# csiro-robotics/ohm

Measured on AMD Instinct MI355X. Metric: rays/sec integrated (occupancy), higher is better.
Workload: dtype f64

## Files before the change

### ohm_amd/csrc/occupancy_math.h

```cpp
#ifndef OHMHIP_OCCUPANCY_MATH_H
#define OHMHIP_OCCUPANCY_MATH_H

#include "walk_device.h"

namespace ohmhip
{
__device__ inline float fInf()
{
  return __int_as_float(0x7f800000);
}

__device__ inline bool sameValue(float a, float b)
{
  return __float_as_uint(a) == __float_as_uint(b);
}

__device__ inline float occMiss(const MapConst &mc, unsigned ray_flags, float initial)
{
  const float inf = fInf();
  const bool unobserved = initial == inf;
  const bool is_free = !unobserved && initial < mc.threshold_value;
  const bool is_occ = !unobserved && initial >= mc.threshold_value;
  float adj = mc.miss_value;
  adj = (unobserved && (ray_flags & OHMHIP_RF_EXCLUDE_UNOBSERVED)) ? inf : adj;
  adj = (is_free && (ray_flags & OHMHIP_RF_EXCLUDE_FREE)) ? 0.0f : adj;
  adj = (is_occ && (ray_flags & OHMHIP_RF_EXCLUDE_OCCUPIED)) ? 0.0f : adj;
  const float base = unobserved ? 0.0f : initial;
  adj = (unobserved || (mc.sat_min < initial && initial < mc.sat_max)) ? adj : 0.0f;
  return (base != inf) ? fmaxf(mc.min_value, base + adj) : base;
}

__device__ inline float occHit(const MapConst &mc, unsigned ray_flags, float initial)
{
  const float inf = fInf();
  const bool unobserved = initial == inf;
  const bool is_free = !unobserved && initial < mc.threshold_value;
  const bool is_occ = !unobserved && initial >= mc.threshold_value;
  float adj = mc.hit_value;
  adj = (unobserved && (ray_flags & OHMHIP_RF_EXCLUDE_UNOBSERVED)) ? inf : adj;
  adj = (is_free && (ray_flags & OHMHIP_RF_EXCLUDE_FREE)) ? 0.0f : adj;
  adj = (is_occ && (ray_flags & OHMHIP_RF_EXCLUDE_OCCUPIED)) ? 0.0f : adj;
  const float base = unobserved ? 0.0f : initial;
  adj = (unobserved || (mc.sat_min < initial && initial < mc.sat_max)) ? adj : 0.0f;
  return (base != inf) ? fminf(base + adj, mc.max_value) : base;
}

__device__ inline float occNullMiss(const MapConst &mc, float initial)
{
  return (initial != fInf()) ? fmaxf(mc.min_value, initial + 0.0f) : initial;
}

__device__ inline float occMissN(const MapConst &mc, unsigned ray_flags, float x, uint32_t n)
{
  constexpr unsigned kExcludeFlags = OHMHIP_RF_EXCLUDE_UNOBSERVED | OHMHIP_RF_EXCLUDE_FREE | OHMHIP_RF_EXCLUDE_OCCUPIED;
  if (n == 0)
  {
    return x;
  }
  if (!(ray_flags & kExcludeFlags))
  {
    const bool unobserved = x == fInf();
    const float base = unobserved ? 0.0f : x;
    const float first_adj = (unobserved || (mc.sat_min < x && x < mc.sat_max)) ? mc.miss_value : 0.0f;
    float nx = fmaxf(mc.min_value, base + first_adj);
    if (nx == x)
    {
      return nx;
    }
    x = nx;
    for (uint32_t k = 1; k < n; ++k)
    {
      const float adj = (mc.sat_min < x && x < mc.sat_max) ? mc.miss_value : 0.0f;
      nx = fmaxf(mc.min_value, x + adj);
      const bool fixed = nx == x;
      x = nx;
      if (fixed)
      {
        break;
      }
    }
    return x;
  }
  for (uint32_t k = 0; k < n; ++k)
  {
    const float nx = occMiss(mc, ray_flags, x);
    const bool fixed = nx == x;
    x = nx;
    if (fixed)
    {
      break;
    }
  }
  return x;
}

__device__ inline uint32_t subVoxelUpdate(uint32_t coord, uint32_t point_count, const double v[3], double resolution)
{
  const int mean_positions = (1 << 10) - 1;
  const double mean_resolution = resolution / double(mean_positions);
  const double offset = double(0.5f) * resolution;
  double mean[3];
  mean[0] = int(coord & mean_positions) * mean_resolution - offset;
  mean[1] = int((coord >> 10) & mean_positions) * mean_resolution - offset;
  mean[2] = int((coord >> 20) & mean_positions) * mean_resolution - offset;
  const double one_on_count_plus_one = double(1) / double(point_count + 1);
  uint32_t pattern = 0;
#pragma unroll
  for (int a = 0; a < 3; ++a)
  {
    mean[a] += (v[a] - mean[a]) * one_on_count_plus_one;
    int pos = pointToRegionCoord(mean[a] + offset, mean_resolution);
    pos = (pos >= 0 ? (pos < (1 << 10) ? pos : mean_positions) : 0);
    pattern |= uint32_t(pos) << (10 * a);
  }
  return pattern | (1u << 31);
}
}

#endif
```

### ohm_amd/csrc/walk_kernel.h

```cpp
#ifndef OHMHIP_WALK_KERNEL_H
#define OHMHIP_WALK_KERNEL_H

#include "batch_scratch.h"
#include "occupancy_math.h"
#include "region_table.h"
#include "walk_device.h"

namespace ohmhip
{
constexpr int kWalkThreads = 1024;
constexpr int kWalkWaves = kWalkThreads / 64;
constexpr int kQueueCap = 128;
#ifndef OHMHIP_LDS_HITS
#define OHMHIP_LDS_HITS 6144
#endif
constexpr int kLdsHits = OHMHIP_LDS_HITS;
constexpr uint32_t kIndexShift = 5;
constexpr uint32_t kIndexBuckets = (1u << kHitVoxelBits) >> kIndexShift;
constexpr int kRefillMinIdle = 20;
constexpr uint32_t kTileFlag = 0x8000u;
constexpr uint32_t kTileCountMask = 0x7fffu;
#ifndef OHMHIP_MAX_CHUNK_SEGMENTS
#define OHMHIP_MAX_CHUNK_SEGMENTS 8192
#endif
constexpr uint32_t kMaxChunkSegments = OHMHIP_MAX_CHUNK_SEGMENTS;
constexpr uint32_t kTraceChunks = 4096;
constexpr uint32_t kTraceWords = 32;
constexpr uint32_t kLengthClasses = 128;

__device__ inline uint32_t tileWord(uint32_t w)
{
  return w ^ (((w >> 5) ^ (w >> 10)) & 31u);
}

__device__ inline uint32_t tileAddress(uint32_t va)
{
  return (va & ~3u) ^ ((((va >> 5) ^ (va >> 10)) & (31u << 2)));
}

__device__ inline void resolveFlaggedMiss(unsigned long long key, const BatchScratch &bs,
                                          const unsigned long long *__restrict__ sorted_hits,
                                          uint32_t *__restrict__ miss_counts, uint32_t *__restrict__ interval_counts,
                                          int region_voxels)
{
  const uint32_t slot = hitSlot(key);
  const uint32_t vi = hitVoxel(key);
  const uint32_t he = bs.info->n_hits;
  uint32_t lo = bs.voxel_first_hit[size_t(slot) * size_t(region_voxels) + vi];
  while (lo < he && hitGroup(sorted_hits[lo]) == hitGroup(key) && sorted_hits[lo] < key)
  {
    ++lo;
  }
  if (lo < he && hitGroup(sorted_hits[lo]) == hitGroup(key))
  {
    atomicAdd(&interval_counts[lo], 1u);
    atomicSub(&miss_counts[size_t(slot) * size_t(region_voxels) + vi], 1u);
  }
}

__device__ inline void flushQueue(const uint2 *queue, uint32_t qcount, unsigned lane, unsigned long long slot_bits,
                                  int ray_shift, bool lds_resolve, const unsigned long long *l_hits,
                                  const uint16_t *l_index, uint32_t n_region_hits, uint32_t *l_intervals,
                                  uint32_t *l_counts,
                                  unsigned long long *__restrict__ events, uint32_t event_capacity,
                                  uint32_t *__restrict__ event_count, int defer_all, const BatchScratch &bs,
                                  const unsigned long long *__restrict__ sorted_hits,
                                  uint32_t *__restrict__ miss_counts, uint32_t *__restrict__ interval_counts,
                                  int region_voxels)
{
  if (lds_resolve)
  {
    for (uint32_t q = lane; q < qcount; q += 64)
    {
      const uint2 e = queue[q];
      const unsigned long long ev =
        slot_bits | ((unsigned long long)e.x << kHitRayBits) | ((unsigned long long)e.y << ray_shift);
      uint32_t lo = l_index[e.x >> kIndexShift], hi = l_index[(e.x >> kIndexShift) + 1u];
      while (lo < hi)
      {
        const uint32_t mid = (lo + hi) >> 1;
        if (l_hits[mid] > ev)
        {
          hi = mid;
        }
        else
        {
          lo = mid + 1;
        }
      }
      if (lo < n_region_hits && hitGroup(l_hits[lo]) == hitGroup(ev))
      {
        atomicAdd(&l_intervals[lo >> 1], 1u << ((lo & 1u) * 16u));
        atomicSub(&l_counts[tileWord(e.x >> 1)], 1u << ((e.x & 1u) * 16u));
      }
    }
    return;
  }
  uint32_t gbase = 0;
  if (lane == 0)
  {
    gbase = atomicAdd(event_count, qcount);
  }
  gbase = __shfl(gbase, 0);
  for (uint32_t q = lane; q < qcount; q += 64)
  {
    const uint2 e = queue[q];
    const unsigned long long ev =
      slot_bits | ((unsigned long long)e.x << kHitRayBits) | ((unsigned long long)e.y << ray_shift);
    if (gbase + q < event_capacity)
    {
      events[gbase + q] = ev;
    }
    else if (!defer_all)
    {
      resolveFlaggedMiss(ev, bs, sorted_hits, miss_counts, interval_counts, region_voxels);
    }
  }
}

constexpr int kFcmpOlt = 4;
constexpr int kIcmpSlt = 40;

__device__ inline int selectI(unsigned long long mask, int if_set, int if_clear)
{
  int r;
  asm("v_cndmask_b32_e64 %0, %1, %2, %3" : "=v"(r) : "v"(if_clear), "v"(if_set), "s"(mask));
  return r;
}

__device__ inline double selectD(unsigned long long mask, double if_set, double if_clear)
{
  const int lo = selectI(mask, __double2loint(if_set), __double2loint(if_clear));
  const int hi = selectI(mask, __double2hiint(if_set), __double2hiint(if_clear));
  return __hiloint2double(hi, lo);
}

__device__ inline int addMask(int value, unsigned long long mask)
{
  asm("v_addc_co_u32_e64 %0, vcc, 0, %0, %1" : "+v"(value) : "s"(mask) : "vcc");
  return value;
}

constexpr int kIcmpEq = 32;
constexpr int kIcmpUlt = 36;

__device__ inline uint32_t selectOrZero(unsigned long long mask, uint32_t if_set)
{
  uint32_t r;
  asm("v_cndmask_b32_e64 %0, 0, %1, %2" : "=v"(r) : "v"(if_set), "s"(mask));
  return r;
}

__device__ inline uint32_t umin3(uint32_t a, uint32_t b, uint32_t c)
{
  uint32_t r;
  asm("v_min3_u32 %0, %1, %2, %3" : "=v"(r) : "v"(a), "v"(b), "v"(c));
  return r;
}

__device__ inline uint32_t umed3(uint32_t a, uint32_t b, uint32_t c)
{
  uint32_t r;
  asm("v_med3_u32 %0, %1, %2, %3" : "=v"(r) : "v"(a), "v"(b), "v"(c));
  return r;
}

__device__ inline uint32_t addSat(uint32_t a, uint32_t b)
{
  uint32_t r;
  asm("v_add_u32_e64 %0, %1, %2 clamp" : "=v"(r) : "v"(a), "v"(b));
  return r;
}

__device__ inline uint32_t addSatUniform(uint32_t a, uint32_t b)
{
  uint32_t r;
  asm("v_add_u32_e64 %0, %1, %2 clamp" : "=v"(r) : "v"(a), "s"(b));
  return r;
}

__device__ inline uint32_t tileAdd(uint32_t byte_address, uint32_t value)
{
  uint32_t old;
  asm volatile("ds_add_rtn_u32 %0, %1, %2" : "=v"(old) : "v"(byte_address), "v"(value) : "memory");
  return old;
}

__device__ inline uint32_t shiftOne(uint32_t shift)
{
  uint32_t r;
  asm("v_lshlrev_b32_e64 %0, %1, 1" : "=v"(r) : "v"(shift));
  return r;
}

__device__ inline uint32_t waitTile(uint32_t old)
{
  asm volatile("s_waitcnt lgkmcnt(0)" : "+v"(old) : : "memory");
  return old;
}

struct WalkArgs
{
  MapConst mc;
  BatchScratch bs;
  const Chunk *chunks;
  const Segment *segments;
  const RayWalk *walks;
  const uint64_t *slot_keys;
  const unsigned long long *sorted_hits;
  const uint32_t *hit_mask;
  uint32_t *miss_counts;
  uint32_t *interval_counts;
  unsigned long long *events;
  uint32_t event_capacity;
  uint32_t *event_count;
  int refill_min_idle;
  unsigned dbg;
  int ray_shift;
  int defer_all;
  float *occupancy;
  unsigned ray_flags;
  unsigned long long *dbg_counters;
  float *tsdf;
  uint32_t *chunk_cursor;
  uint32_t n_chunks;
  int rewalk;
  int flag_all;
  int inline_hits;
};

constexpr uint32_t kWalkCursorWords = 24;
#ifndef OHMHIP_WALK_UNROLL
#define OHMHIP_WALK_UNROLL 2
#endif
constexpr int kWalkUnroll = OHMHIP_WALK_UNROLL;

template <int kThreadsT, int kTileVoxelsT, int kLdsHitsT, uint32_t kSegmentsT, int kQueueCapT, int kMinWavesPerEuT>
struct WalkGeometry
{
  static constexpr int kMinWavesPerEu = kMinWavesPerEuT;
  static constexpr int kThreads = kThreadsT;
  static constexpr int kWaves = kThreadsT / 64;
  static constexpr int kTileVoxels = kTileVoxelsT;
  static constexpr int kLdsHits = kLdsHitsT;
  static constexpr uint32_t kSegments = kSegmentsT;
  static constexpr int kQueueCap = kQueueCapT;
};
using WalkFull = WalkGeometry<kWalkThreads, 1 << kHitVoxelBits, kLdsHits, kMaxChunkSegments, kQueueCap, 1>;
using WalkHalf = WalkGeometry<kWalkThreads / 2, (1 << kHitVoxelBits) / 2, kLdsHits / 2, kMaxChunkSegments / 2, 96, 4>;
template <bool kSpecial, bool kTrace, typename G = WalkFull>
__global__ void __launch_bounds__(G::kThreads, G::kMinWavesPerEu) k_region_walk(WalkArgs args)
{
  extern __shared__ __attribute__((aligned(16))) uint32_t lds[];
  const MapConst &mc = args.mc;
  const uint32_t count_words = uint32_t(mc.region_voxels + 1) >> 1;
  const uint32_t mask_words = uint32_t(mc.region_voxels + 31) >> 5;
  uint32_t *l_counts = lds;
  uint2 *l_queues = reinterpret_cast<uint2 *>(lds + ((count_words + 31u) & ~31u));
  unsigned long long *l_hits = reinterpret_cast<unsigned long long *>(l_queues + G::kWaves * G::kQueueCap);
  uint32_t *l_intervals = reinterpret_cast<uint32_t *>(l_hits + G::kLdsHits);
  uint32_t *l_cursor = l_intervals + G::kLdsHits / 2;
  uint32_t *l_hist = l_cursor + kWalkCursorWords;
  uint32_t *l_idle = l_hist + kLengthClasses;
  uint16_t *l_index = reinterpret_cast<uint16_t *>(l_idle + 64);
  uint16_t *l_order = l_index + kIndexBuckets + 2;

  const int defer_all = args.defer_all;
  auto fetchNextChunk = [&](uint32_t *record, bool first = false) {
    const uint32_t next = first ? blockIdx.x : gridDim.x + atomicAdd(args.chunk_cursor, 1u);
    record[1] = next;
    if (next < args.n_chunks)
    {
      const Chunk c = args.chunks[next];
      record[2] = c.slot;
      record[3] = c.seg_begin;
      record[4] = c.seg_end;
      record[5] = c.hash_index;
      record[6] = defer_all ? 0u : args.bs.hit_begin[c.slot];
      record[7] = defer_all ? 0u : args.bs.hit_end[c.slot];
      const uint64_t key = args.slot_keys[c.slot];
      record[8] = uint32_t(key);
      record[9] = uint32_t(key >> 32);
    }
  };
  constexpr int kSegPerThread = int(G::kSegments) / G::kThreads;
  constexpr int kHitsPerThread = G::kLdsHits / uint32_t(G::kThreads);
  struct ChunkRecord
  {
    uint32_t index, slot, seg_begin, seg_end, hash_index, hb, he, key_lo, key_hi;
  };
  auto readRecord = [&](const uint32_t *record) {
    ChunkRecord r;
    r.index = __builtin_amdgcn_readfirstlane(record[1]);
    r.slot = __builtin_amdgcn_readfirstlane(record[2]);
    r.seg_begin = __builtin_amdgcn_readfirstlane(record[3]);
    r.seg_end = __builtin_amdgcn_readfirstlane(record[4]);
    r.hash_index = __builtin_amdgcn_readfirstlane(record[5]);
    r.hb = __builtin_amdgcn_readfirstlane(record[6]);
    r.he = __builtin_amdgcn_readfirstlane(record[7]);
    r.key_lo = __builtin_amdgcn_readfirstlane(record[8]);
    r.key_hi = __builtin_amdgcn_readfirstlane(record[9]);
    return r;
  };
  unsigned long long pf_hits[kHitsPerThread] = {};
  uint32_t pf_vox[kSegPerThread] = {};
  uint32_t pf_mask = 0;
  auto prefetchChunk = [&](const ChunkRecord &r) {
    const uint32_t n_hits = r.he - r.hb;
    if (!defer_all && n_hits && n_hits <= uint32_t(G::kLdsHits))
    {
#pragma unroll
      for (int j = 0; j < kHitsPerThread; ++j)
      {
        pf_hits[j] = args.sorted_hits[r.hb + min(threadIdx.x + uint32_t(j) * uint32_t(G::kThreads), n_hits - 1u)];
      }
    }
    pf_mask = args.hit_mask[size_t(r.slot) * mask_words + min(threadIdx.x, mask_words - 1u)];
    const uint32_t n = r.seg_end - r.seg_begin;
#pragma unroll
    for (int j = 0; j < kSegPerThread; ++j)
    {
      pf_vox[j] = args.segments[r.seg_begin + min(threadIdx.x + uint32_t(j) * uint32_t(G::kThreads), n - 1u)].vox;
    }
  };
  if (threadIdx.x == 0 || threadIdx.x == 64)
  {
    fetchNextChunk(l_cursor + (threadIdx.x ? kWalkCursorWords / 2 : 0), threadIdx.x == 0);
  }
  __syncthreads();
  ChunkRecord cur = readRecord(l_cursor);
  ChunkRecord next = readRecord(l_cursor + kWalkCursorWords / 2);
  if (next.index < cur.index)
  {
    const ChunkRecord swap = cur;
    cur = next;
    next = swap;
  }
  if (cur.index < args.n_chunks)
  {
    prefetchChunk(cur);
  }
  __syncthreads();
  while (cur.index < args.n_chunks)
  {
    unsigned long long clk_start = 0;
    if (kTrace)
    {
      clk_start = wall_clock64();
    }
    const uint32_t chunk_index = cur.index;
    Chunk chunk;
    chunk.slot = cur.slot;
    chunk.seg_begin = cur.seg_begin;
    chunk.seg_end = cur.seg_end;
    chunk.hash_index = cur.hash_index;
    const uint32_t hb = cur.hb;
    const uint32_t he = cur.he;
    const int region_x = int(int16_t(cur.key_lo & 0xffffu));
    const int region_y = int(int16_t(cur.key_lo >> 16));
    const int region_z = int(int16_t(cur.key_hi & 0xffffu));
    const uint32_t n_seg = chunk.seg_end - chunk.seg_begin;
    const Segment *chunk_segments = args.segments + chunk.seg_begin;

    const uint32_t n_region_hits = he - hb;
    const bool lds_resolve = !defer_all && n_region_hits <= uint32_t(G::kLdsHits);
    unsigned long long my_hits[kHitsPerThread];
#pragma unroll
    for (int j = 0; j < kHitsPerThread; ++j)
    {
      my_hits[j] = pf_hits[j];
    }
    const uint32_t *g_mask = args.hit_mask + size_t(chunk.slot) * mask_words;
    const uint32_t my_mask = pf_mask;
    uint32_t lens[kSegPerThread];
#pragma unroll
    for (int j = 0; j < kSegPerThread; ++j)
    {
      lens[j] = min(pf_vox[j] >> kSegVoxelBits, kLengthClasses - 1u);
    }
    if (threadIdx.x < kLengthClasses)
    {
      l_hist[threadIdx.x] = 0;
    }
    if (threadIdx.x == 0)
    {
      l_cursor[0] = 0;
    }
    if (threadIdx.x < 64)
    {
      l_idle[threadIdx.x] = 0;
    }
    const bool stamp = kTrace && threadIdx.x == 0;
    unsigned long long clk_p[6] = { 0, 0, 0, 0, 0, 0 };
    if (stamp)
    {
      clk_p[0] = wall_clock64();
    }
    for (uint32_t w = threadIdx.x; w < mask_words; w += uint32_t(G::kThreads))
    {
      const uint32_t mword = args.flag_all ? 0xffffffffu : ((w == threadIdx.x) ? my_mask : g_mask[w]);
      const uint32_t swizzle = tileWord(w * 16u) ^ (w * 16u);
#pragma unroll
      for (uint32_t q = 0; q < 4; ++q)
      {
        const uint32_t logical = w * 16u + q * 4u;
        if (logical + 3u < count_words)
        {
          uint32_t v[4];
#pragma unroll
          for (uint32_t r = 0; r < 4; ++r)
          {
            const uint32_t two = (mword >> ((q * 4u + (r ^ (swizzle & 3u))) * 2u)) & 3u;
            v[r] = ((two & 1u) << 15) | ((two & 2u) << 30);
          }
          *reinterpret_cast<uint4 *>(&l_counts[logical ^ (swizzle & ~3u)]) = make_uint4(v[0], v[1], v[2], v[3]);
        }
        else
        {
          for (uint32_t r = 0; r < 4; ++r)
          {
            if (logical + r < count_words)
            {
              const uint32_t two = (mword >> ((q * 4u + r) * 2u)) & 3u;
              l_counts[tileWord(logical + r)] = ((two & 1u) << 15) | ((two & 2u) << 30);
            }
          }
        }
      }
    }
    if (stamp)
    {
      clk_p[1] = wall_clock64();
    }
    __syncthreads();
    bool prefetched = false;
    if (stamp)
    {
      clk_p[2] = wall_clock64();
    }
#pragma unroll
    for (int j = 0; j < kSegPerThread; ++j)
    {
      if (threadIdx.x + uint32_t(j) * uint32_t(G::kThreads) < n_seg)
      {
        atomicAdd(&l_hist[lens[j]], 1u);
      }
    }
    if (lds_resolve && n_region_hits)
    {
#pragma unroll
      for (int j = 0; j < kHitsPerThread; ++j)
      {
        const uint32_t i = threadIdx.x + uint32_t(j) * uint32_t(G::kThreads);
        if (i < n_region_hits)
        {
          l_hits[i] = my_hits[j];
        }
        if (i < (n_region_hits + 1) / 2)
        {
          l_intervals[i] = 0;
        }
      }
    }
    __syncthreads();
    if (stamp)
    {
      clk_p[3] = wall_clock64();
    }
    if (lds_resolve && n_region_hits)
    {
#pragma unroll
      for (int j = 0; j < kHitsPerThread; ++j)
      {
        const uint32_t i = threadIdx.x + uint32_t(j) * uint32_t(G::kThreads);
        if (i < n_region_hits)
        {
          auto bucketOf = [](unsigned long long key) {
            return (uint32_t(key >> kHitRayBits) & ((1u << kHitVoxelBits) - 1u)) >> kIndexShift;
          };
          const uint32_t b = bucketOf(my_hits[j]);
          const uint32_t first = (i == 0) ? 0u : bucketOf(l_hits[i - 1]) + 1u;
          for (uint32_t k = first; k <= b; ++k)
          {
            l_index[k] = uint16_t(i);
          }
          if (i + 1 == n_region_hits)
          {
            for (uint32_t k = b + 1u; k <= kIndexBuckets; ++k)
            {
              l_index[k] = uint16_t(n_region_hits);
            }
          }
        }
      }
    }
    if (threadIdx.x < 64)
    {
      const uint32_t hi_class = kLengthClasses - 1u - 2u * threadIdx.x;
      const uint32_t a = l_hist[hi_class];
      const uint32_t b = l_hist[hi_class - 1u];
      uint32_t incl = a + b;
#pragma unroll
      for (int d = 1; d < 64; d <<= 1)
      {
        const uint32_t up = __shfl_up(incl, d);
        incl += (int(threadIdx.x) >= d) ? up : 0u;
      }
      const uint32_t excl = incl - (a + b);
      l_hist[hi_class] = excl;
      l_hist[hi_class - 1u] = excl + a;
    }
    __syncthreads();
#pragma unroll
    for (int j = 0; j < kSegPerThread; ++j)
    {
      const uint32_t i = threadIdx.x + uint32_t(j) * uint32_t(G::kThreads);
      if (i < n_seg)
      {
        l_order[atomicAdd(&l_hist[lens[j]], 1u)] = uint16_t(i);
      }
    }
    __syncthreads();
    if (stamp)
    {
      clk_p[4] = wall_clock64();
      if (chunk_index < kTraceChunks)
      {
        unsigned long long *rec = args.dbg_counters + 16 + size_t(chunk_index) * kTraceWords;
        rec[20] = clk_p[0];
        rec[21] = clk_p[1];
        rec[22] = clk_p[2];
        rec[23] = clk_p[3];
      }
    }

    const unsigned lane = laneId();
    const unsigned wave = threadIdx.x >> 6;
    uint2 *queue = l_queues + wave * G::kQueueCap;
    const int dimx = mc.dim[0];
    const int dimxy = mc.dim[0] * mc.dim[1];
    const unsigned long long slot_bits = (unsigned long long)chunk.slot << kHitSlotShift;
    const int ray_shift = args.ray_shift;
    const int refill_min_idle = args.refill_min_idle;
    const bool refill_only = kTrace && (args.dbg & 16u) != 0;
    const uint32_t fix_margin = mc.fix_margin;
    const uint32_t idle_address = uint32_t(reinterpret_cast<char *>(l_idle + lane) - reinterpret_cast<char *>(lds));

    int left = 0;
    uint32_t f0 = 0, f1 = 0, f2 = 0, d0 = 0, d1 = 0, d2 = 0;
    int sx = 0, sy = 0, sz = 0;
    uint32_t va = 0;
    uint32_t ray = 0;
    uint32_t skip = 0;
    uint32_t end_last = 0;
    uint32_t qcount = 0;
    bool exhausted = false;
    uint32_t dbg_iters = 0, dbg_active = 0, dbg_refills = 0, dbg_fm = 0, dbg_slow = 0;
    uint32_t dbg_s2 = 0, dbg_s3 = 0, dbg_sl = 0, dbg_sp = 0;
    unsigned long long clk_loop = 0;
    if (kTrace)
    {
      clk_loop = wall_clock64();
    }

    int refill_threshold = refill_min_idle;
    while (true)
    {
      const unsigned long long am = __ballot(left > 0);
      const int n_idle = 64 - __popcll(am);
      if (__builtin_expect(n_idle >= refill_threshold, 0))
      {
        if (exhausted)
        {
          break;
        }
        if (kTrace)
        {
          ++dbg_refills;
        }
        uint32_t base = 0;
        if (lane == 0)
        {
          base = atomicAdd(l_cursor, uint32_t(n_idle));
        }
        base = __builtin_amdgcn_readfirstlane(base);
        exhausted = base + uint32_t(n_idle) >= n_seg;
        refill_threshold = exhausted ? 64 : refill_threshold;
        const unsigned long long idle = ~am;
        const uint32_t mine =
          base + __builtin_amdgcn_mbcnt_hi(uint32_t(idle >> 32), __builtin_amdgcn_mbcnt_lo(uint32_t(idle), 0u));
        if (left <= 0 && mine < n_seg)
        {
          const uint4 *rec = reinterpret_cast<const uint4 *>(chunk_segments + l_order[mine]);
          const uint4 ra = rec[0];
          const uint4 rb = rec[1];
          f0 = ra.x;
          f1 = ra.y;
          f2 = ra.z;
          va = (ra.w & ((1u << kSegVoxelBits) - 1u)) << 1;
          left = int(ra.w >> kSegVoxelBits);
          d0 = rb.x & ~kSegNegative;
          d1 = rb.y & ~kSegNegative;
          d2 = rb.z & ~kSegNegative;
          sx = (rb.x & kSegNegative) ? -2 : 2;
          sy = (rb.y & kSegNegative) ? -2 * dimx : 2 * dimx;
          sz = (rb.z & kSegNegative) ? -2 * dimxy : 2 * dimxy;
          ray = rb.w & kSegRayMask;
          if (kSpecial)
          {
            skip = (rb.w & kSegSkipFirst) ? 1u : 0u;
            end_last = (rb.w & kSegEnd) ? 1u : 0u;
          }
          left = refill_only ? 0 : left;
        }
        if (!prefetched)
        {
          prefetched = true;
          if (next.index < args.n_chunks)
          {
            prefetchChunk(next);
          }
        }
      }

      uint32_t olds[kWalkUnroll];
      uint32_t visited[kWalkUnroll];
#pragma unroll
      for (int u = 0; u < kWalkUnroll; ++u)
      {
        const bool at_end = kSpecial && end_last && left == 1;
        const bool visit = kSpecial ? (left > 0 && (at_end || !skip)) : (left > 0);
        visited[u] = va;
        olds[u] = tileAdd(visit ? tileAddress(va) : idle_address, shiftOne(va << 3));
        if (kSpecial)
        {
          skip = 0;
        }
        if (kTrace)
        {
          ++dbg_iters;
          dbg_active += uint32_t(__popcll(__ballot(visit)));
        }

        int stride;
        {
          const uint32_t fmin = umin3(f0, f1, f2);
          const uint32_t fmed = umed3(f0, f1, f2);
          const uint32_t limit = min(fmed, kFixMaxDelta);
          const uint32_t lead = addSatUniform(fmin, fix_margin);
          const unsigned long long certain = __builtin_amdgcn_uicmp(lead, limit, kIcmpUlt);
          unsigned long long a0 = __builtin_amdgcn_uicmp(f0, fmin, kIcmpEq);
          unsigned long long a2 = __builtin_amdgcn_uicmp(f2, fmin, kIcmpEq);
          const unsigned long long slow = __ballot(left > 1) & ~certain;
          if (__builtin_expect(slow != 0, 0))
          {
            int axis = 1;
            if ((slow >> lane) & 1ull)
            {
              uint32_t r = ray;
              asm volatile("" : "+v"(r));
              axis = exactNextAxis(mc, args.walks[r], region_x, region_y, region_z, va >> 1);
            }
            a0 = (a0 & ~slow) | (slow & __ballot(axis == 0));
            a2 = (a2 & ~slow) | (slow & __ballot(axis == 2));
            if (kTrace)
            {
              ++dbg_slow;
              dbg_s2 += uint32_t(__popcll(slow & __ballot(left == 2)));
              dbg_s3 += uint32_t(__popcll(slow & __ballot(left == 3)));
              dbg_sl += uint32_t(__popcll(slow));
              dbg_sp += uint32_t(__popcll(slow & __ballot((d0 | d1 | d2) == 0u)));
            }
          }
          const unsigned long long a1 = ~(a0 | a2);
          f0 = addSat(f0, selectOrZero(a0, d0));
          f1 = addSat(f1, selectOrZero(a1, d1));
          f2 = addSat(f2, selectOrZero(a2, d2));
          stride = selectI(a2, sz, selectI(a0, sx, sy));
        }
        va += uint32_t(stride);
        left -= 1;
      }

      __builtin_amdgcn_sched_barrier(0);
#pragma unroll
      for (int u = 0; u < kWalkUnroll; ++u)
      {
        olds[u] = waitTile(olds[u]);
      }
#pragma unroll
      for (int u = 0; u < kWalkUnroll; ++u)
      {
        const bool flagged = __builtin_amdgcn_ubfe(olds[u], (visited[u] << 3) | 15u, 1u) != 0;
        const unsigned long long fm = __ballot(flagged);
        if (kTrace)
        {
          dbg_fm += fm ? 1u : 0u;
        }
        if (fm)
        {
          if (flagged)
          {
            const uint32_t pos =
              qcount + __builtin_amdgcn_mbcnt_hi(uint32_t(fm >> 32), __builtin_amdgcn_mbcnt_lo(uint32_t(fm), 0u));
            queue[pos] = make_uint2(visited[u] >> 1, ray);
          }
          qcount += uint32_t(__popcll(fm));
          if (qcount > uint32_t(G::kQueueCap - 64))
          {
            flushQueue(queue, qcount, lane, slot_bits, ray_shift, lds_resolve, l_hits, l_index, n_region_hits,
                       l_intervals, l_counts, args.events, args.event_capacity, args.event_count, defer_all, args.bs,
                       args.sorted_hits, args.miss_counts, args.interval_counts, mc.region_voxels);
            qcount = 0;
          }
        }
      }
    }

    if (kTrace && lane == 0)
    {
      const unsigned long long clk_end_loop = wall_clock64();
      if (chunk_index < kTraceChunks)
      {
        unsigned long long *rec = args.dbg_counters + 16 + size_t(chunk_index) * kTraceWords;
        if (wave < 15)
        {
          rec[2 + wave] = clk_end_loop;
        }
        if (wave == 0)
        {
          rec[0] = n_seg | ((unsigned long long)((chunk.hash_index >> 31) & 1u) << 32);
          rec[1] = clk_loop;
          rec[18] = clk_start;
          rec[17] = (unsigned long long)__builtin_amdgcn_s_getreg(63492) |
                    ((unsigned long long)__builtin_amdgcn_s_getreg(63508) << 32);
        }
      }
      if (args.dbg & 128u)
      {
        atomicAdd(&args.dbg_counters[0], (unsigned long long)dbg_iters);
        atomicAdd(&args.dbg_counters[1], (unsigned long long)dbg_active);
        atomicAdd(&args.dbg_counters[2], (unsigned long long)dbg_refills);
        atomicAdd(&args.dbg_counters[3], (unsigned long long)dbg_fm);
        atomicAdd(&args.dbg_counters[4], (unsigned long long)dbg_slow);
        atomicAdd(&args.dbg_counters[5], (unsigned long long)dbg_s2);
        atomicAdd(&args.dbg_counters[6], (unsigned long long)dbg_s3);
        atomicAdd(&args.dbg_counters[7], (unsigned long long)dbg_sl);
        atomicAdd(&args.dbg_counters[8], (unsigned long long)dbg_sp);
      }
    }
    if (qcount)
    {
      flushQueue(queue, qcount, lane, slot_bits, ray_shift, lds_resolve, l_hits, l_index, n_region_hits, l_intervals,
                 l_counts, args.events, args.event_capacity, args.event_count, defer_all, args.bs, args.sorted_hits,
                 args.miss_counts, args.interval_counts, mc.region_voxels);
    }
    if (threadIdx.x == 0)
    {
      fetchNextChunk(l_cursor);
    }
    __syncthreads();
    const ChunkRecord after_next = readRecord(l_cursor);
    if (stamp && chunk_index < kTraceChunks)
    {
      args.dbg_counters[16 + size_t(chunk_index) * kTraceWords + 24] = wall_clock64();
    }

    const bool inline_hits = args.inline_hits && lds_resolve && n_region_hits > 0u && args.occupancy && !args.rewalk &&
                             (chunk.hash_index & 0x80000000u);
    if (lds_resolve && !inline_hits)
    {
      for (uint32_t i = threadIdx.x; i < n_region_hits; i += uint32_t(G::kThreads))
      {
        const uint32_t c = (l_intervals[i >> 1] >> ((i & 1u) * 16u)) & 0xffffu;
        if (c)
        {
          atomicAdd(&args.interval_counts[hb + i], c);
        }
      }
    }
    uint32_t *g_counts = args.miss_counts + size_t(chunk.slot) * size_t(mc.region_voxels);
    if (args.rewalk && (chunk.hash_index & 0x80000000u))
    {
      __syncthreads();
      cur = next;
      next = after_next;
      continue;
    }
    if (args.occupancy && (chunk.hash_index & 0x80000000u))
    {
      float *g_occ = args.occupancy + size_t(chunk.slot) * size_t(mc.region_voxels);
      constexpr uint32_t kWordsPerThread = uint32_t(G::kTileVoxels) / 2u / uint32_t(G::kThreads) / 2u;
      const bool even_voxels = (mc.region_voxels & 1) == 0;
      for (uint32_t half = 0; half < 2u; ++half)
      {
      uint32_t words[kWordsPerThread];
      float2 values[kWordsPerThread];
#pragma unroll
      for (uint32_t j = 0; j < kWordsPerThread; ++j)
      {
        const uint32_t i = threadIdx.x + (half * kWordsPerThread + j) * uint32_t(G::kThreads);
        const uint32_t flagged_w = (i < count_words) ? l_counts[tileWord(i)] : 0u;
        uint32_t w = flagged_w;
        w = (w & kTileFlag) ? (w & 0xffff0000u) : w;
        w = (w & (kTileFlag << 16)) ? (w & 0x0000ffffu) : w;
        if (!defer_all && !inline_hits)
        {
          if ((flagged_w & kTileFlag) && (flagged_w & kTileCountMask))
          {
            atomicAdd(&g_counts[2 * i], flagged_w & kTileCountMask);
          }
          if ((flagged_w & (kTileFlag << 16)) && ((flagged_w >> 16) & kTileCountMask))
          {
            atomicAdd(&g_counts[2 * i + 1], (flagged_w >> 16) & kTileCountMask);
          }
        }
        words[j] = w;
        values[j] = make_float2(0.0f, 0.0f);
        if (w)
        {
          if (even_voxels)
          {
            values[j] = *reinterpret_cast<const float2 *>(&g_occ[2 * i]);
          }
          else
          {
            values[j].x = g_occ[2 * i];
            values[j].y = (2 * i + 1 < uint32_t(mc.region_voxels)) ? g_occ[2 * i + 1] : 0.0f;
          }
        }
      }
#pragma unroll
      for (uint32_t j = 0; j < kWordsPerThread; ++j)
      {
        const uint32_t i = threadIdx.x + (half * kWordsPerThread + j) * uint32_t(G::kThreads);
        const uint32_t w = words[j];
        if (w)
        {
          const uint32_t n0 = w & kTileCountMask;
          const uint32_t n1 = (w >> 16) & kTileCountMask;
          if (n0)
          {
            const float v = occMissN(mc, args.ray_flags, values[j].x, n0);
            if (!sameValue(v, values[j].x))
            {
              g_occ[2 * i] = v;
            }
          }
          if (n1)
          {
            const float v = occMissN(mc, args.ray_flags, values[j].y, n1);
            if (!sameValue(v, values[j].y))
            {
              g_occ[2 * i + 1] = v;
            }
          }
        }
      }
      if (stamp && chunk_index < kTraceChunks)
      {
        args.dbg_counters[16 + size_t(chunk_index) * kTraceWords + 25 + half] = wall_clock64();
      }
      }
      if (inline_hits)
      {
        for (uint32_t i = threadIdx.x; i < n_region_hits; i += uint32_t(G::kThreads))
        {
          const unsigned long long key = l_hits[i];
          const unsigned long long group = key >> kHitRayBits;
          if (i > 0u && (l_hits[i - 1u] >> kHitRayBits) == group)
          {
            continue;
          }
          const uint32_t vi = uint32_t(group) & ((1u << kHitVoxelBits) - 1u);
          float x = g_occ[vi];
          for (uint32_t j = i; j < n_region_hits && (l_hits[j] >> kHitRayBits) == group; ++j)
          {
            x = occMissN(mc, args.ray_flags, x, (l_intervals[j >> 1] >> ((j & 1u) * 16u)) & 0xffffu);
            x = occHit(mc, args.ray_flags, x);
          }
          const uint32_t w = l_counts[tileWord(vi >> 1)];
          x = occMissN(mc, args.ray_flags, x, (w >> ((vi & 1u) * 16u)) & kTileCountMask);
          g_occ[vi] = x;
        }
        if (stamp && chunk_index < kTraceChunks)
        {
          args.dbg_counters[16 + size_t(chunk_index) * kTraceWords + 27] = wall_clock64();
        }
        if (threadIdx.x == 0)
        {
          atomicOr(&args.bs.hit_begin[chunk.slot], kSamplesApplied);
        }
      }
      if (stamp && chunk_index < kTraceChunks)
      {
        args.dbg_counters[16 + size_t(chunk_index) * kTraceWords + 19] = wall_clock64();
      }
      __syncthreads();
      cur = next;
      next = after_next;
      continue;
    }
    if (args.tsdf && (chunk.hash_index & 0x80000000u))
    {
      float2 *g_tsdf = reinterpret_cast<float2 *>(args.tsdf) + size_t(chunk.slot) * size_t(mc.region_voxels);
      constexpr uint32_t kTsdfBatch = 4;
      for (uint32_t first = threadIdx.x; first < count_words; first += kTsdfBatch * uint32_t(G::kThreads))
      {
        uint32_t words[kTsdfBatch];
        float2 values[2 * kTsdfBatch];
#pragma unroll
        for (uint32_t j = 0; j < kTsdfBatch; ++j)
        {
          const uint32_t i = first + j * uint32_t(G::kThreads);
          uint32_t w = (i < count_words) ? l_counts[tileWord(i)] : 0u;
          w = (w & kTileFlag) ? (w & 0xffff0000u) : w;
          w = (w & (kTileFlag << 16)) ? (w & 0x0000ffffu) : w;
          words[j] = w;
          values[2 * j] = make_float2(0.0f, 0.0f);
          values[2 * j + 1] = make_float2(0.0f, 0.0f);
          if (w & kTileCountMask)
          {
            values[2 * j] = g_tsdf[2 * i];
          }
          if ((w >> 16) & kTileCountMask)
          {
            values[2 * j + 1] = g_tsdf[2 * i + 1];
          }
        }
#pragma unroll
        for (uint32_t j = 0; j < kTsdfBatch; ++j)
        {
          const uint32_t i = first + j * uint32_t(G::kThreads);
          const uint32_t n0 = words[j] & kTileCountMask;
          const uint32_t n1 = (words[j] >> 16) & kTileCountMask;
          if (n0)
          {
            const float wn = values[2 * j].x + float(n0);
            g_tsdf[2 * i] = make_float2((mc.tsdf_max_weight < wn) ? mc.tsdf_max_weight : wn, mc.tsdf_trunc);
          }
          if (n1)
          {
            const float wn = values[2 * j + 1].x + float(n1);
            g_tsdf[2 * i + 1] = make_float2((mc.tsdf_max_weight < wn) ? mc.tsdf_max_weight : wn, mc.tsdf_trunc);
          }
        }
      }
      if (stamp && chunk_index < kTraceChunks)
      {
        args.dbg_counters[16 + size_t(chunk_index) * kTraceWords + 19] = wall_clock64();
      }
      __syncthreads();
      cur = next;
      next = after_next;
      continue;
    }
    for (uint32_t i = threadIdx.x; i < count_words; i += uint32_t(G::kThreads))
    {
      const uint32_t w = l_counts[tileWord(i)];
      if (w & (kTileCountMask | (kTileCountMask << 16)))
      {
#pragma unroll
        for (uint32_t half = 0; half < 2; ++half)
        {
          const uint32_t entry = (w >> (16u * half)) & 0xffffu;
          const uint32_t n = entry & kTileCountMask;
          if (n && !(defer_all && (entry & kTileFlag)))
          {
            atomicAdd(&g_counts[2 * i + half], n);
          }
        }
      }
    }
    if (stamp && chunk_index < kTraceChunks)
    {
      args.dbg_counters[16 + size_t(chunk_index) * kTraceWords + 19] = wall_clock64();
    }
    __syncthreads();
    cur = next;
    next = after_next;
  }
}

__global__ void __launch_bounds__(256)
  k_flagged_events(BatchScratch bs, const unsigned long long *__restrict__ events, uint32_t event_capacity,
                   const uint32_t *__restrict__ event_count, const unsigned long long *__restrict__ sorted_hits,
                   uint32_t *__restrict__ miss_counts, uint32_t *__restrict__ interval_counts, int region_voxels,
                   uint32_t *__restrict__ host_event_count)
{
  if (blockIdx.x == 0 && threadIdx.x == 0)
  {
    *host_event_count = *event_count;
  }
  const uint32_t n = min(*event_count, event_capacity);
  const uint32_t stride = gridDim.x * blockDim.x;
  for (uint32_t i = blockIdx.x * blockDim.x + threadIdx.x; i < n; i += stride)
  {
    resolveFlaggedMiss(events[i], bs, sorted_hits, miss_counts, interval_counts, region_voxels);
  }
}
}

#endif
```

Measured before the change: 1.220 billion.

## Add specialized full-tile apply/flush paths and spread length-class histogram across copies

Adds noinline specialised routines for full-size region tiles. One applies the miss updates with wave-uniform pointers and constants, ballot-guarded atomics and batched LDS reads. The other flushes the count tile in unrolled bursts instead of a strided loop. The segment-length histogram is split into 8 per-lane copies aliased onto the queue LDS area, with a new vectorised scan, to cut LDS atomic contention during ordering. This adds code size, call overhead from the noinline functions, and a larger scan in exchange for fewer divergent branches and less atomic contention.

```diff
diff --git a/ohm_amd/csrc/occupancy_math.h b/ohm_amd/csrc/occupancy_math.h
--- a/ohm_amd/csrc/occupancy_math.h
+++ b/ohm_amd/csrc/occupancy_math.h
@@ -94,6 +94,40 @@
   return x;
 }
 
+struct MissConst
+{
+  float miss_value, min_value, sat_min, sat_max;
+};
+
+__device__ inline float occMissNPlainWave(const MissConst mc, float x, uint32_t n)
+{
+  const bool unobserved = x == fInf();
+  const float base = unobserved ? 0.0f : x;
+  const bool first_moves = unobserved | ((mc.sat_min < x) & (x < mc.sat_max));
+  const float first_adj = first_moves ? mc.miss_value : 0.0f;
+  float nx = fmaxf(mc.min_value, base + first_adj);
+  const bool repeat = (n > 1u) & !(nx == x);
+  if (__ballot(repeat))
+  {
+    if (repeat)
+    {
+      float cur = nx;
+      for (uint32_t k = 1; k < n; ++k)
+      {
+        const float adj = (mc.sat_min < cur && cur < mc.sat_max) ? mc.miss_value : 0.0f;
+        nx = fmaxf(mc.min_value, cur + adj);
+        const bool fixed = nx == cur;
+        cur = nx;
+        if (fixed)
+        {
+          break;
+        }
+      }
+    }
+  }
+  return n ? nx : x;
+}
+
 __device__ inline uint32_t subVoxelUpdate(uint32_t coord, uint32_t point_count, const double v[3], double resolution)
 {
   const int mean_positions = (1 << 10) - 1;
diff --git a/ohm_amd/csrc/walk_kernel.h b/ohm_amd/csrc/walk_kernel.h
--- a/ohm_amd/csrc/walk_kernel.h
+++ b/ohm_amd/csrc/walk_kernel.h
@@ -27,6 +27,8 @@
 constexpr uint32_t kTraceChunks = 4096;
 constexpr uint32_t kTraceWords = 32;
 constexpr uint32_t kLengthClasses = 128;
+constexpr uint32_t kOrderCopies = 8;
+constexpr uint32_t kOrderBins = kLengthClasses * kOrderCopies;
 
 __device__ inline uint32_t tileWord(uint32_t w)
 {
@@ -248,6 +250,176 @@
 };
 using WalkFull = WalkGeometry<kWalkThreads, 1 << kHitVoxelBits, kLdsHits, kMaxChunkSegments, kQueueCap, 1>;
 using WalkHalf = WalkGeometry<kWalkThreads / 2, (1 << kHitVoxelBits) / 2, kLdsHits / 2, kMaxChunkSegments / 2, 96, 4>;
+using LdsWord = __attribute__((address_space(3))) uint32_t;
+using GlobalWord = __attribute__((address_space(1))) uint32_t;
+using GlobalByte = __attribute__((address_space(1))) char;
+using GlobalFloat = __attribute__((address_space(1))) float;
+typedef float Float2 __attribute__((ext_vector_type(2)));
+typedef uint32_t Quad __attribute__((ext_vector_type(4)));
+using GlobalFloat2 = __attribute__((address_space(1))) Float2;
+using LdsQuad = __attribute__((address_space(3))) Quad;
+
+__device__ inline void addGlobal(GlobalWord *address, uint32_t value)
+{
+  __hip_atomic_fetch_add(address, value, __ATOMIC_RELAXED, __HIP_MEMORY_SCOPE_AGENT);
+}
+
+template <typename T>
+__device__ inline T *uniformPointer(T *p)
+{
+  const unsigned long long v = reinterpret_cast<unsigned long long>(p);
+  const uint32_t lo = __builtin_amdgcn_readfirstlane(uint32_t(v));
+  const uint32_t hi = __builtin_amdgcn_readfirstlane(uint32_t(v >> 32));
+  return reinterpret_cast<T *>(((unsigned long long)hi << 32) | lo);
+}
+
+__device__ inline float uniformFloat(float v)
+{
+  return __uint_as_float(__builtin_amdgcn_readfirstlane(__float_as_uint(v)));
+}
+
+__device__ __noinline__ void scanOrderBins(LdsWord *bins, uint32_t lane)
+{
+  constexpr uint32_t kQuads = kOrderBins / 256u;
+  LdsQuad *mine = reinterpret_cast<LdsQuad *>(bins) + lane * kQuads;
+  Quad c[kQuads];
+  uint32_t total = 0;
+#pragma unroll
+  for (uint32_t q = 0; q < kQuads; ++q)
+  {
+    c[q] = mine[q];
+    total += c[q].x + c[q].y + c[q].z + c[q].w;
+  }
+  uint32_t incl = total;
+#pragma unroll
+  for (int d = 1; d < 64; d <<= 1)
+  {
+    const uint32_t up = __shfl_up(incl, d);
+    incl += (int(lane) >= d) ? up : 0u;
+  }
+  uint32_t run = incl - total;
+#pragma unroll
+  for (uint32_t q = 0; q < kQuads; ++q)
+  {
+    Quad e;
+    e.x = run;
+    e.y = e.x + c[q].x;
+    e.z = e.y + c[q].y;
+    e.w = e.z + c[q].z;
+    run = e.w + c[q].w;
+    mine[q] = e;
+  }
+}
+
+template <typename G>
+__device__ __noinline__ void applyFullTile(const LdsWord *tile, float *occupancy, uint32_t *g_counts, MissConst mc,
+                                           unsigned long long *stamps)
+{
+  constexpr uint32_t kWordsPerThread = uint32_t(G::kTileVoxels) / 2u / uint32_t(G::kThreads) / 2u;
+  GlobalByte *occ_bytes = (GlobalByte *)uniformPointer(occupancy);
+  GlobalWord *counts = (GlobalWord *)uniformPointer(g_counts);
+  stamps = uniformPointer(stamps);
+  mc.miss_value = uniformFloat(mc.miss_value);
+  mc.min_value = uniformFloat(mc.min_value);
+  mc.sat_min = uniformFloat(mc.sat_min);
+  mc.sat_max = uniformFloat(mc.sat_max);
+  for (uint32_t half = 0; half < 2u; ++half)
+  {
+    const uint32_t first = threadIdx.x + half * kWordsPerThread * uint32_t(G::kThreads);
+    uint32_t words[kWordsPerThread];
+    Float2 values[kWordsPerThread];
+#pragma unroll
+    for (uint32_t j = 0; j < kWordsPerThread; ++j)
+    {
+      words[j] = tile[tileWord(first + j * uint32_t(G::kThreads))];
+    }
+#pragma unroll
+    for (uint32_t j = 0; j < kWordsPerThread; ++j)
+    {
+      const uint32_t i = first + j * uint32_t(G::kThreads);
+      const uint32_t sampled = ((words[j] >> 15) & 0x00010001u) * 0xffffu;
+      const uint32_t kept = words[j] & sampled & (kTileCountMask | (kTileCountMask << 16));
+      words[j] &= ~sampled;
+      if (counts && __ballot(kept != 0u))
+      {
+        if (kept & 0xffffu)
+        {
+          addGlobal(&counts[2 * i], kept & 0xffffu);
+        }
+        if (kept >> 16)
+        {
+          addGlobal(&counts[2 * i + 1], kept >> 16);
+        }
+      }
+      values[j] = Float2(0.0f);
+      if (words[j])
+      {
+        values[j] = *(const GlobalFloat2 *)(occ_bytes + i * 8u);
+      }
+    }
+#pragma unroll
+    for (uint32_t j = 0; j < kWordsPerThread; ++j)
+    {
+      const uint32_t i = first + j * uint32_t(G::kThreads);
+      if (__ballot(words[j] != 0u))
+      {
+        const float v0 = occMissNPlainWave(mc, values[j].x, words[j] & 0xffffu);
+        if (!sameValue(v0, values[j].x))
+        {
+          *(GlobalFloat *)(occ_bytes + i * 8u) = v0;
+        }
+        const float v1 = occMissNPlainWave(mc, values[j].y, words[j] >> 16);
+        if (!sameValue(v1, values[j].y))
+        {
+          *(GlobalFloat *)(occ_bytes + i * 8u + 4u) = v1;
+        }
+      }
+    }
+    if (stamps && threadIdx.x == 0)
+    {
+      stamps[half] = wall_clock64();
+    }
+  }
+}
+
+template <typename G>
+__device__ __noinline__ void flushFullTile(const LdsWord *tile, uint32_t *g_counts, uint32_t skip_masked)
+{
+  constexpr uint32_t kBurst = 8;
+  constexpr uint32_t kWords = uint32_t(G::kTileVoxels) / 2u / uint32_t(G::kThreads);
+  static_assert(kWords % kBurst == 0u, "the tile flush reads whole bursts");
+  GlobalWord *counts = (GlobalWord *)uniformPointer(g_counts);
+  skip_masked = __builtin_amdgcn_readfirstlane(skip_masked);
+  for (uint32_t burst = 0; burst < kWords / kBurst; ++burst)
+  {
+    const uint32_t first = threadIdx.x + burst * kBurst * uint32_t(G::kThreads);
+    uint32_t words[kBurst];
+#pragma unroll
+    for (uint32_t j = 0; j < kBurst; ++j)
+    {
+      words[j] = tile[tileWord(first + j * uint32_t(G::kThreads))];
+    }
+#pragma unroll
+    for (uint32_t j = 0; j < kBurst; ++j)
+    {
+      const uint32_t i = first + j * uint32_t(G::kThreads);
+      const uint32_t masked = skip_masked ? ((words[j] >> 15) & 0x00010001u) * 0xffffu : 0u;
+      const uint32_t n = words[j] & ~masked & (kTileCountMask | (kTileCountMask << 16));
+      if (__ballot(n != 0u))
+      {
+        if (n & 0xffffu)
+        {
+          addGlobal(&counts[2 * i], n & 0xffffu);
+        }
+        if (n >> 16)
+        {
+          addGlobal(&counts[2 * i + 1], n >> 16);
+        }
+      }
+    }
+  }
+}
+
 template <bool kSpecial, bool kTrace, typename G = WalkFull>
 __global__ void __launch_bounds__(G::kThreads, G::kMinWavesPerEu) k_region_walk(WalkArgs args)
 {
@@ -260,10 +432,12 @@
   unsigned long long *l_hits = reinterpret_cast<unsigned long long *>(l_queues + G::kWaves * G::kQueueCap);
   uint32_t *l_intervals = reinterpret_cast<uint32_t *>(l_hits + G::kLdsHits);
   uint32_t *l_cursor = l_intervals + G::kLdsHits / 2;
-  uint32_t *l_hist = l_cursor + kWalkCursorWords;
-  uint32_t *l_idle = l_hist + kLengthClasses;
+  uint32_t *l_idle = l_cursor + kWalkCursorWords + kLengthClasses;
   uint16_t *l_index = reinterpret_cast<uint16_t *>(l_idle + 64);
   uint16_t *l_order = l_index + kIndexBuckets + 2;
+  uint32_t *l_bins = reinterpret_cast<uint32_t *>(l_queues);
+  static_assert(kOrderBins <= 2u * uint32_t(G::kWaves) * uint32_t(G::kQueueCap), "the class counters alias the queues");
+  static_assert(kOrderBins % 256u == 0u, "the scan gives each of 64 lanes whole uint4s");
 
   const int defer_all = args.defer_all;
   auto fetchNextChunk = [&](uint32_t *record, bool first = false) {
@@ -372,15 +546,16 @@
     }
     const uint32_t *g_mask = args.hit_mask + size_t(chunk.slot) * mask_words;
     const uint32_t my_mask = pf_mask;
-    uint32_t lens[kSegPerThread];
+    uint32_t bins[kSegPerThread];
 #pragma unroll
     for (int j = 0; j < kSegPerThread; ++j)
     {
-      lens[j] = min(pf_vox[j] >> kSegVoxelBits, kLengthClasses - 1u);
-    }
-    if (threadIdx.x < kLengthClasses)
-    {
-      l_hist[threadIdx.x] = 0;
+      bins[j] = (kLengthClasses - 1u - min(pf_vox[j] >> kSegVoxelBits, kLengthClasses - 1u)) * kOrderCopies +
+                (threadIdx.x & (kOrderCopies - 1u));
+    }
+    for (uint32_t b = threadIdx.x; b < kOrderBins; b += uint32_t(G::kThreads))
+    {
+      l_bins[b] = 0;
     }
     if (threadIdx.x == 0)
     {
@@ -443,7 +618,7 @@
     {
       if (threadIdx.x + uint32_t(j) * uint32_t(G::kThreads) < n_seg)
       {
-        atomicAdd(&l_hist[lens[j]], 1u);
+        atomicAdd(&l_bins[bins[j]], 1u);
       }
     }
     if (lds_resolve && n_region_hits)
@@ -496,19 +671,7 @@
     }
     if (threadIdx.x < 64)
     {
-      const uint32_t hi_class = kLengthClasses - 1u - 2u * threadIdx.x;
-      const uint32_t a = l_hist[hi_class];
-      const uint32_t b = l_hist[hi_class - 1u];
-      uint32_t incl = a + b;
-#pragma unroll
-      for (int d = 1; d < 64; d <<= 1)
-      {
-        const uint32_t up = __shfl_up(incl, d);
-        incl += (int(threadIdx.x) >= d) ? up : 0u;
-      }
-      const uint32_t excl = incl - (a + b);
-      l_hist[hi_class] = excl;
-      l_hist[hi_class - 1u] = excl + a;
+      scanOrderBins((LdsWord *)l_bins, threadIdx.x);
     }
     __syncthreads();
 #pragma unroll
@@ -517,7 +680,7 @@
       const uint32_t i = threadIdx.x + uint32_t(j) * uint32_t(G::kThreads);
       if (i < n_seg)
       {
-        l_order[atomicAdd(&l_hist[lens[j]], 1u)] = uint16_t(i);
+        l_order[atomicAdd(&l_bins[bins[j]], 1u)] = uint16_t(i);
       }
     }
     __syncthreads();
@@ -792,6 +955,18 @@
       float *g_occ = args.occupancy + size_t(chunk.slot) * size_t(mc.region_voxels);
       constexpr uint32_t kWordsPerThread = uint32_t(G::kTileVoxels) / 2u / uint32_t(G::kThreads) / 2u;
       const bool even_voxels = (mc.region_voxels & 1) == 0;
+      constexpr unsigned kExcludeFlags =
+        OHMHIP_RF_EXCLUDE_UNOBSERVED | OHMHIP_RF_EXCLUDE_FREE | OHMHIP_RF_EXCLUDE_OCCUPIED;
+      if (!defer_all && !(args.ray_flags & kExcludeFlags) && mc.region_voxels == G::kTileVoxels)
+      {
+        const MissConst miss = { mc.miss_value, mc.min_value, mc.sat_min, mc.sat_max };
+        applyFullTile<G>((const LdsWord *)l_counts, g_occ, inline_hits ? nullptr : g_counts, miss,
+                         (kTrace && chunk_index < kTraceChunks) ?
+                           args.dbg_counters + 16 + size_t(chunk_index) * kTraceWords + 25 :
+                           nullptr);
+      }
+      else
+      {
       for (uint32_t half = 0; half < 2u; ++half)
       {
       uint32_t words[kWordsPerThread];
@@ -860,6 +1035,7 @@
       if (stamp && chunk_index < kTraceChunks)
       {
         args.dbg_counters[16 + size_t(chunk_index) * kTraceWords + 25 + half] = wall_clock64();
+      }
       }
       }
       if (inline_hits)
@@ -955,7 +1131,12 @@
       next = after_next;
       continue;
     }
-    for (uint32_t i = threadIdx.x; i < count_words; i += uint32_t(G::kThreads))
+    const bool full_tile = mc.region_voxels == G::kTileVoxels;
+    if (full_tile)
+    {
+      flushFullTile<G>((const LdsWord *)l_counts, g_counts, uint32_t(defer_all));
+    }
+    for (uint32_t i = threadIdx.x; !full_tile && i < count_words; i += uint32_t(G::kThreads))
     {
       const uint32_t w = l_counts[tileWord(i)];
       if (w & (kTileCountMask | (kTileCountMask << 16)))
```

After: 1.271 billion (median of 6 runs). +4.2%, better.
